# jurmy24/orb-slam3-rust

Measured on AMD Instinct MI355X. Metric: stereo frames/sec ORB extract+match @752x480, higher is better.
Workload: dtype u8; 1 GPU; Synthetic 752x480 stereo, 2000 ORB/frame, extract+match+triangulate (BASELINE configs[1]); n_features=2000, batch_pairs_per_gpu=512, distinct_batches=3, unique_pairs=1536, parallelism=frames sharded, 1 rank(s), no collective

## Files before the change

orb-slam3-rust_amd/csrc/orb_kernels.hip:

```cpp
#include <cfloat>
#include <cmath>

#include "orbx_internal.hpp"

namespace {

#include "orb_pattern_31.inc"

constexpr int EDGE = 31;

__constant__ __attribute__((aligned(16))) signed char c_pattern[256 * 4];

struct XcdMap { unsigned per_img, magic; };
__device__ __forceinline__ bool xcd_decode_at(XcdMap m, int n_img, unsigned L, int& img, int& b) {
  const unsigned x = L & 7u, slot = L >> 3;
  unsigned grp = __umulhi(slot, m.magic);
  unsigned r = slot - grp * m.per_img;
  if (r >= m.per_img) { ++grp; r -= m.per_img; }
  b = (int)r;
  img = (int)(grp * 8u + x);
  return img < n_img;
}
__device__ __forceinline__ bool xcd_decode(XcdMap m, int n_img, int& img, int& b) { return xcd_decode_at(m, n_img, blockIdx.x, img, b); }
static inline XcdMap xcd_map(int per_img) {
// ... 5 lines not shown
                                                    int& pitch) {
  if (l == 0) { pitch = s.l0_pitch; return s.l0 + (size_t)img * s.l0_img_stride; }
  pitch = g.lv[l].pitch;
  return s.pyr + (size_t)img * g.slot_bytes + g.lv[l].off;
}

__global__ __launch_bounds__(256) void copy_l0_kernel(const uint8_t* __restrict__ src, size_t img_stride,
                                                      size_t row_stride, int w, int h, uint8_t* __restrict__ pyr,
                                                      unsigned slot, int pitch) {
  const int img = blockIdx.z;
  const int y = blockIdx.y;
  const uint8_t* s = src + (size_t)img * img_stride + (size_t)y * row_stride;
  uint8_t* d = pyr + (size_t)img * slot + (size_t)y * pitch;
  for (int x = blockIdx.x * 256 + threadIdx.x; x < w; x += gridDim.x * 256) d[x] = s[x];
}

__device__ __forceinline__ unsigned ld_u32(const uint8_t* p);
#ifndef ORBX_RESIZE_ROWS
#define ORBX_RESIZE_ROWS 6
#endif
constexpr int RESIZE_ROWS = ORBX_RESIZE_ROWS;
__device__ __forceinline__ unsigned pack_byte2(unsigned a, unsigned b, unsigned c, unsigned d) {
  return __builtin_amdgcn_perm(b, a, 0x0c0c0602u) | __builtin_amdgcn_perm(d, c, 0x06020c0cu);
}

__device__ __forceinline__ unsigned resize_h(unsigned long long win, int o, unsigned coef) {
  const unsigned pr = (unsigned)(win >> (8 * o));
  return __builtin_amdgcn_udot4(pr, coef, pr & 0xffu, false);
}

constexpr int RZ_LP = 128;
constexpr int rz_src_rows(int rows) { return (16 * rows - 1) * 3 / 2 + 3; }
constexpr int RESIZE_ROWS_SMALL = 2;
#ifndef ORBX_RESIZE_CHAIN
#define ORBX_RESIZE_CHAIN 1
#endif
constexpr int RESIZE_CHAIN = ORBX_RESIZE_CHAIN;
template <int RESIZE_ROWS>
__global__ __launch_bounds__(256) void resize_kernel(OrbSrc s, OrbGeom g, int l, int n_img, XcdMap xm, int tiles_x, int n_tiles,
                                                     const unsigned* __restrict__ xtab,
                                                     const unsigned* __restrict__ ytab) {
  constexpr int RZ_SRC_ROWS = rz_src_rows(RESIZE_ROWS);
  __shared__ __attribute__((aligned(16))) uint8_t st[RZ_SRC_ROWS * RZ_LP + 16];
  int img, chain;
  if (!xcd_decode(xm, n_img, img, chain)) return;
  int sp;
  const uint8_t* src = level_ptr(s, g, img, l - 1, sp);
  const int sh = g.lv[l - 1].h;
  const int w = g.lv[l].w, h = g.lv[l].h, dp = g.lv[l].pitch;
  uint8_t* dst = s.pyr + (size_t)img * g.slot_bytes + g.lv[l].off;
  const int tid = threadIdx.x;
  constexpr int NP = (RZ_SRC_ROWS + 31) / 32;
  struct Tile { int X0, Y0, ax, ncol, sy_lo, nrow, off; };
  uint4 v[NP];
  auto fetch = [&](int tb, Tile& t) {
    const int tby = tb / tiles_x, tbx = tb - tby * tiles_x;
    t.X0 = tbx * 64; t.Y0 = tby * (16 * RESIZE_ROWS);
    const int sx_lo = (int)(xtab[t.X0] >> 16);
    const int xb_last = min((int)(xtab[min(t.X0 + 60, ((w + 3) & ~3) - 4)] >> 16), sp - 8);
    t.ax = min(sx_lo & ~15, sp - 16);
    t.ncol = (xb_last + 8 - t.ax + 15) >> 4;
    t.sy_lo = (int)(ytab[t.Y0] >> 16);
    const int sy_hi = min((int)(ytab[min(t.Y0 + 16 * RESIZE_ROWS - 1, h - 1)] >> 16) + 1, sh - 1);
    t.nrow = sy_hi - t.sy_lo + 1;
    const int c = tid & 7;
    const int cs = min(t.ax + 16 * c, sp - 16);
    t.off = cs - t.ax;
    const uint8_t* gp = src + (unsigned)(__umul24((unsigned)(t.sy_lo + (tid >> 3)), (unsigned)sp) + (unsigned)cs);
    const unsigned gstep = 32u * (unsigned)sp;
#pragma unroll
    for (int k = 0; k < NP; ++k)
      if (c < t.ncol && (tid >> 3) + 32 * k < t.nrow) __builtin_memcpy(&v[k], gp + (unsigned)k * gstep, 16);
  };
  const int tb0 = chain * RESIZE_CHAIN, tb_end = min(tb0 + RESIZE_CHAIN, n_tiles);
  Tile cur, nxt;
  fetch(tb0, cur);
  for (int tb = tb0; tb < tb_end; ++tb) {
    const int x0 = cur.X0 + (tid & 15) * 4;
    const int yb = cur.Y0 + (tid >> 4);
    const bool active = yb < h && x0 < w;
    uint4 xt4 = {0u, 0u, 0u, 0u};
    unsigned yt[RESIZE_ROWS];
    if (active) {
      xt4 = *reinterpret_cast<const uint4*>(xtab + x0);
#pragma unroll
      for (int r = 0; r < RESIZE_ROWS; ++r) yt[r] = ytab[min(yb + 16 * r, h - 1)];
    }
#pragma unroll
    for (int k = 0; k < NP; ++k) {
      const int r = (tid >> 3) + 32 * k;
      if ((tid & 7) < cur.ncol && r < cur.nrow) {
        if ((cur.off & 15) == 0) *reinterpret_cast<uint4*>(&st[r * RZ_LP + cur.off]) = v[k];
        else {
          unsigned* q = reinterpret_cast<unsigned*>(&st[r * RZ_LP + cur.off]);
          q[0] = v[k].x; q[1] = v[k].y; q[2] = v[k].z; q[3] = v[k].w;
        }
      }
    }
    __syncthreads();
    if (tb + 1 < tb_end) fetch(tb + 1, nxt);
    if (active) {
      const unsigned xt[4] = {xt4.x, xt4.y, xt4.z, xt4.w};
      const int xb = min((int)(xt[0] >> 16), sp - 8);
      const int col = xb - cur.ax, sh8 = col & 3;
      const uint8_t* lp = st + (col & ~3);
#pragma unroll
      for (int r = 0; r < RESIZE_ROWS; ++r) {
        const int y = yb + 16 * r;
        if (y >= h) break;
        const int y0 = (int)(yt[r] >> 16), y1 = min(y0 + 1, sh - 1);
        const unsigned* p0 = reinterpret_cast<const unsigned*>(lp + (y0 - cur.sy_lo) * RZ_LP);
        const unsigned* p1 = reinterpret_cast<const unsigned*>(lp + (y1 - cur.sy_lo) * RZ_LP);
        const unsigned a0 = p0[0], a1 = p0[1], a2 = p0[2], b0 = p1[0], b1 = p1[1], b2 = p1[2];
        const unsigned long long w0 = (unsigned long long)__builtin_amdgcn_alignbyte(a1, a0, (unsigned)sh8) |
                                      ((unsigned long long)__builtin_amdgcn_alignbyte(a2, a1, (unsigned)sh8) << 32);
        const unsigned long long w1 = (unsigned long long)__builtin_amdgcn_alignbyte(b1, b0, (unsigned)sh8) |
                                      ((unsigned long long)__builtin_amdgcn_alignbyte(b2, b1, (unsigned)sh8) << 32);
        const unsigned cy1 = yt[r] & 0xffffu, cy0 = 256u - cy1;
        unsigned vv[4];
#pragma unroll
        for (int k = 0; k < 4; ++k) {
          const int o = (int)(xt[k] >> 16) - xb;
          const unsigned cx1 = xt[k] & 0xffffu;
          const unsigned coef = (255u - cx1) | (cx1 << 8);
          const unsigned h0 = resize_h(w0, o, coef), h1 = resize_h(w1, o, coef);
          vv[k] = __umul24(cy0, h0) + __umul24(cy1, h1) + 32768u;
        }
        const unsigned packed = pack_byte2(vv[0], vv[1], vv[2], vv[3]);
        *reinterpret_cast<unsigned*>(dst + (unsigned)(__umul24((unsigned)y, (unsigned)dp) + (unsigned)x0)) = packed;
      }
    }
    __syncthreads();
    cur = nxt;
  }
}

__device__ __forceinline__ void decode_tile(const unsigned* __restrict__ tab, int tile, int& l, int& tx, int& ty) {
  const unsigned e = tab[tile];
  l = (int)(e & 7u); tx = (int)((e >> 3) & 0x3fffu); ty = (int)(e >> 17);
}


#ifndef ORBX_BLUR_PF
#define ORBX_BLUR_PF 2
#endif
constexpr int BLUR_PF = ORBX_BLUR_PF;
#ifndef ORBX_BLUR_STRIP
#define ORBX_BLUR_STRIP 32
#endif
#if defined(ORBX_BLUR_NOARITH) && ORBX_BLUR_NOARITH == 2
constexpr int BLUR_W = 256, BLUR_HALO = 0;
#else
constexpr int BLUR_W = 248, BLUR_HALO = 1;
#endif
constexpr int BLUR_STRIP = ORBX_BLUR_STRIP, BLUR_H = 4 * BLUR_STRIP;

__device__ __forceinline__ void blur_hsum(unsigned d0, unsigned d1, unsigned d2, unsigned (&hs)[4]) {
  const unsigned G0 = 18u | (34u << 8) | (48u << 16) | (56u << 24);
  const unsigned G1 = 48u | (34u << 8) | (18u << 16);
  hs[0] = __builtin_amdgcn_udot4(__builtin_amdgcn_alignbyte(d2, d1, 1), G1,
                                 __builtin_amdgcn_udot4(__builtin_amdgcn_alignbyte(d1, d0, 1), G0, 0u, false), false);
  hs[1] = __builtin_amdgcn_udot4(__builtin_amdgcn_alignbyte(d2, d1, 2), G1,
                                 __builtin_amdgcn_udot4(__builtin_amdgcn_alignbyte(d1, d0, 2), G0, 0u, false), false);
  hs[2] = __builtin_amdgcn_udot4(__builtin_amdgcn_alignbyte(d2, d1, 3), G1,
                                 __builtin_amdgcn_udot4(__builtin_amdgcn_alignbyte(d1, d0, 3), G0, 0u, false), false);
  hs[3] = __builtin_amdgcn_udot4(d2, G1, __builtin_amdgcn_udot4(d1, G0, 0u, false), false);
}
// ... 473 lines not shown
  __syncthreads();
  for (int q = tid; q < npos; q += FT_THREADS) {
    const int p = s_pos[q];
    const int j = p >> 6, i = p & 63;
    const int x = x0 + i - 1, y = y0 + j - 1;
    const int sc = ss[j][i];
    const bool corner = sc > 0 && i >= 1 && i <= FT_W && j >= 1 && j <= FT_H && x < w - EDGE && y < h - EDGE;
    if (corner) {
      const int m = max(max(max((int)ss[j - 1][i - 1], (int)ss[j - 1][i]), max((int)ss[j - 1][i + 1], (int)ss[j][i - 1])),
                        max(max((int)ss[j][i + 1], (int)ss[j + 1][i - 1]), max((int)ss[j + 1][i], (int)ss[j + 1][i + 1])));
      if (sc > m) {
        const int pos = atomicAdd(&s_cnt, 1);
        if (pos < FAST_LIST_CAP) s_list[pos] = ((unsigned)sc << 24) | ((unsigned)y << 12) | (unsigned)x;
        else atomicOr(status, ORBX_ST_INTERNAL);
      }
    }
  }
  __syncthreads();
  acc_cnt = min(s_cnt, FAST_LIST_CAP);
  acc_il = img * g.n_levels + l;
  acc_off = g.lv[l].cand_off;
  acc_cap = g.lv[l].cand_cap;
  cur = nxt;
  }
  if (acc_cnt > 0) append();
}

__device__ __forceinline__ unsigned ld_u32(const uint8_t* p) {
  unsigned v;
  __builtin_memcpy(&v, p, 4);
  return v;
}

__device__ __forceinline__ float harris_response(const uint8_t* __restrict__ img, int pitch, int x0, int y0) {
  int a = 0, b = 0, c = 0;
  int rowm[9], row0[9], rowp[9];
  unsigned w[9][3];
#ifdef ORBX_HARRIS_UNALIGNED
  const uint8_t* p = img + (size_t)(y0 - 4) * pitch + (x0 - 4);
#pragma unroll
  for (int r = 0; r < 9; ++r) {
    const uint8_t* pr = p + (size_t)r * pitch;
    w[r][0] = ld_u32(pr); w[r][1] = ld_u32(pr + 4); w[r][2] = ld_u32(pr + 8);
  }
#else
  const unsigned sh = (unsigned)(x0 - 4) & 3u;
  const uint8_t* p = img + (unsigned)(__umul24((unsigned)(y0 - 4), (unsigned)pitch) + ((unsigned)(x0 - 4) & ~3u));
  struct alignas(4) Row12 { unsigned d[3]; };
  Row12 rw[9];
#pragma unroll
  for (int r = 0; r < 9; ++r) rw[r] = *reinterpret_cast<const Row12*>(p + (unsigned)r * (unsigned)pitch);
#pragma unroll
  for (int r = 0; r < 9; ++r) {
    w[r][0] = __builtin_amdgcn_alignbyte(rw[r].d[1], rw[r].d[0], sh);
    w[r][1] = __builtin_amdgcn_alignbyte(rw[r].d[2], rw[r].d[1], sh);
    w[r][2] = rw[r].d[2] >> (8u * sh);
  }
#endif
#define ORBX_ROW(dst, r)                                                                    \
  _Pragma("unroll") for (int k = 0; k < 4; ++k) {                                             \
    dst[k] = (int)((w[r][0] >> (8 * k)) & 0xffu);                                             \
    dst[4 + k] = (int)((w[r][1] >> (8 * k)) & 0xffu);                                         \
  }                                                                                           \
  dst[8] = (int)(w[r][2] & 0xffu);
  ORBX_ROW(rowm, 0)
  ORBX_ROW(row0, 1)
#pragma unroll
  for (int i = 0; i < 7; ++i) {
    ORBX_ROW(rowp, i + 2)
#pragma unroll
    for (int j = 0; j < 7; ++j) {
      const int Ix = (row0[j + 2] - row0[j]) * 2 + (rowm[j + 2] - rowm[j]) + (rowp[j + 2] - rowp[j]);
      const int Iy = (rowp[j + 1] - rowm[j + 1]) * 2 + (rowp[j] - rowm[j]) + (rowp[j + 2] - rowm[j + 2]);
      a += Ix * Ix; b += Iy * Iy; c += Ix * Iy;
    }
#pragma unroll
    for (int k = 0; k < 9; ++k) { rowm[k] = row0[k]; row0[k] = rowp[k]; }
  }
#undef ORBX_ROW
  const float scale = 1.f / (4 * 7 * 255.f);
  const float scale_sq_sq = scale * scale * scale * scale;
  const float fa = (float)a, fb = (float)b, fc = (float)c;
  const float t1 = __fmul_rn(fa, fb);
  const float t2 = __fmul_rn(fc, fc);
  const float sm = __fadd_rn(fa, fb);
  const float t3 = __fmul_rn(__fmul_rn(0.04f, sm), sm);
  float r = __fmul_rn(__fsub_rn(__fsub_rn(t1, t2), t3), scale_sq_sq);
  if (r == 0.f) r = 0.f;
  return r;
}

__device__ __forceinline__ unsigned orderable(float f) {
  const unsigned u = __float_as_uint(f);
  return (u & 0x80000000u) ? ~u : (u | 0x80000000u);
}
__device__ __forceinline__ float from_orderable(unsigned o) {
  const unsigned u = (o & 0x80000000u) ? (o & 0x7fffffffu) : ~o;
  return __uint_as_float(u);
}

struct HarrisPlan { int start[ORBX_MAX_LEVELS + 1]; };
__global__ __launch_bounds__(256) void harris_select_kernel(OrbSrc s, OrbGeom g, int n_img, XcdMap xm, const unsigned* __restrict__ cand,
                                                            const unsigned* __restrict__ cand_count,
                                                            const unsigned* __restrict__ hist,
                                                            unsigned long long* __restrict__ sel,
                                                            unsigned* __restrict__ sel_count, HarrisPlan hp) {
  __shared__ unsigned sh[256];
  __shared__ int s_thr;
  int img, bb;
  if (!xcd_decode(xm, n_img, img, bb)) return;
  int l = 0;
#pragma unroll
  for (int k = 1; k < ORBX_MAX_LEVELS; ++k) l += (bb >= hp.start[k]) ? 1 : 0;
  const int chunk = bb - hp.start[l], n_chunks = hp.start[l + 1] - hp.start[l];
  const int il = img * g.n_levels + l;
  const int tid = threadIdx.x;
  const unsigned count = min(cand_count[il], g.lv[l].cand_cap);
  const unsigned want = 2u * (unsigned)g.lv[l].quota;
  {
    const int lane = tid & 63, wave = tid >> 6;
    const unsigned hv = hist[(size_t)il * 256 + tid];
    const int incl = wave_scan_incl((int)hv);
    unsigned suf = (unsigned)(__builtin_amdgcn_readlane(incl, 63) - incl) + hv;
    if (lane == 0) sh[wave] = suf;
    if (tid == 0) s_thr = 0;
    __syncthreads();
    for (int w2 = wave + 1; w2 < 4; ++w2) suf += sh[w2];
    const unsigned long long m = __ballot(suf >= want);
    if (want == 0) { if (tid == 0) s_thr = 256; }
    else if (count > want && m && lane == 0) atomicMax(&s_thr, wave * 64 + 63 - __clzll((long long)m));
    __syncthreads();
  }
  const unsigned thr = (unsigned)s_thr;
  int pitch;
  const uint8_t* src = level_ptr(s, g, img, l, pitch);
  const unsigned* cl = cand + (size_t)img * g.cand_total + g.lv[l].cand_off;
  unsigned long long* out = sel + (size_t)img * g.cand_total + g.lv[l].cand_off;
  __shared__ unsigned s_pass[1024];
  __shared__ unsigned s_np;
  const int lane = tid & 63;
  const unsigned per = (count + (unsigned)n_chunks - 1u) / (unsigned)n_chunks;
  const unsigned lim = min(count, (chunk + 1) * per);
  for (unsigned base = chunk * per; base < lim; base += 1024u) {
    if (tid == 0) s_np = 0;
    __syncthreads();
#pragma unroll
    for (int k = 0; k < 4; ++k) {
      const unsigned i = base + k * 256 + tid;
      const unsigned c = i < lim ? cl[i] : 0u;
      const bool pass = i < lim && (c >> 24) >= thr;
      const unsigned long long m = __ballot(pass);
      if (m) {
        unsigned p0 = 0;
        if (lane == 0) p0 = (unsigned)lds_add_rtn(reinterpret_cast<int*>(&s_np), __popcll(m));
        p0 = __builtin_amdgcn_readfirstlane(p0);
        if (pass) s_pass[p0 + __builtin_amdgcn_mbcnt_hi((unsigned)(m >> 32), __builtin_amdgcn_mbcnt_lo((unsigned)m, 0u))] = c;
      }
    }
    __syncthreads();
    const unsigned np = s_np;
    unsigned mine = 0;
    for (unsigned q0 = (unsigned)(tid & ~63); q0 < np; q0 += 256) mine += min(64u, np - q0);
    unsigned pos0 = 0;
    if (lane == 0 && mine) pos0 = atomicAdd(&sel_count[il], mine);
    for (unsigned q0 = 0; q0 < np; q0 += 256) {
      const unsigned q = q0 + tid;
      if (q < np) {
        const unsigned c = s_pass[q];
        const int x = (int)(c & 0xfffu), y = (int)((c >> 12) & 0xfffu);
        const float r = harris_response(src, pitch, x, y);
        const unsigned long long key = ((unsigned long long)(~orderable(r)) << 32) | ((unsigned)y << 16) | (unsigned)x;
        out[__builtin_amdgcn_readfirstlane(pos0) + (q0 >> 8) * 64u + (unsigned)lane] = key;
      }
    }
    __syncthreads();
  }
}

constexpr int RK_NT = 256;
#ifndef ORBX_RK_CAP
#define ORBX_RK_CAP 1024
#endif
constexpr int RK_CAP = ORBX_RK_CAP;
static_assert(RK_CAP == 1024 || RK_CAP == 2048, "a power of two, at least the 1024 counters the tile sort keeps in the array, at most the 2048 keys held in registers");
template <int E>
__device__ __forceinline__ void rank_pass(const unsigned long long* __restrict__ in, unsigned long long* __restrict__ out,
                                          unsigned M, unsigned g0, unsigned long long* chunk, int quota, unsigned* s_thr) {
  constexpr int CH = RK_CAP;
  const int tid = threadIdx.x;
  unsigned long long my[E];
  unsigned rank[E];
#pragma unroll
  for (int e = 0; e < E; ++e) {
    const unsigned idx = g0 + e * RK_NT + tid;
    my[e] = idx < M ? in[idx] : ~0ull;
    rank[e] = 0;
  }
  for (unsigned c0 = 0; c0 < M; c0 += CH) {
    const unsigned n = min((unsigned)CH, M - c0);
    __syncthreads();
    for (unsigned i = tid; i < n; i += RK_NT) chunk[i] = in[c0 + i];
    __syncthreads();
    for (unsigned k = 0; k < n; ++k) {
      const unsigned long long v = chunk[k];
#pragma unroll
      for (int e = 0; e < E; ++e) rank[e] += (v < my[e]) ? 1u : 0u;
// ... 581 lines not shown
      for (int mb = 0; mb < 4; ++mb) a1[mb] = anx[mb] ^ (df_i4){(int)0x80808080u, (int)0x80808080u, (int)0x80808080u, (int)0x80808080u};
      if (wi + 4 < nwin) fetch(wi + 4, anx);
      unsigned char* out0 = s_tile + (unsigned)((c - ox + m16) * DT_PITCH + (r - oy) + 4 * q);
#pragma unroll
      for (int nb = 0; nb < 3; ++nb) {
        const df_i4 t1 = band[64 * nb];
        df_i4 hh[4];
#pragma unroll
        for (int mb = 0; mb < 4; ++mb) hh[mb] = __builtin_amdgcn_mfma_i32_16x16x64_i8(a1[mb], t1, (df_i4){0, 0, 0, 0}, 0, 0, 0);
        df_i4 bhi, blo;
#pragma unroll
        for (int mb = 0; mb < 4; ++mb) {
          const unsigned p01 = __builtin_amdgcn_perm((unsigned)hh[mb][1], (unsigned)hh[mb][0], 0x05010400u);
          const unsigned p23 = __builtin_amdgcn_perm((unsigned)hh[mb][3], (unsigned)hh[mb][2], 0x05010400u);
          blo[mb] = (int)(__builtin_amdgcn_perm(p23, p01, 0x05040100u) ^ 0x80808080u);
          bhi[mb] = (int)__builtin_amdgcn_perm(p23, p01, 0x07060302u);
        }
#pragma unroll
        for (int mb2 = 0; mb2 < 3; ++mb2) {
          const df_i4 t2 = band[64 * (3 + mb2)];
          const df_i4 shi = __builtin_amdgcn_mfma_i32_16x16x64_i8(t2, bhi, (df_i4){0, 0, 0, 0}, 0, 0, 0);
          const df_i4 slo = __builtin_amdgcn_mfma_i32_16x16x64_i8(t2, blo, (df_i4){8454144, 8454144, 8454144, 8454144}, 0, 0, 0);
          const unsigned v0 = ((unsigned)shi[0] << 8) + (unsigned)slo[0], v1 = ((unsigned)shi[1] << 8) + (unsigned)slo[1];
          const unsigned v2 = ((unsigned)shi[2] << 8) + (unsigned)slo[2], v3 = ((unsigned)shi[3] << 8) + (unsigned)slo[3];
          const unsigned u01 = __builtin_amdgcn_perm(v1, v0, 0x00000602u), u23 = __builtin_amdgcn_perm(v3, v2, 0x00000602u);
          *reinterpret_cast<unsigned*>(out0 + (16 * nb) * DT_PITCH + 16 * mb2) = __builtin_amdgcn_perm(u23, u01, 0x05040100u);
        }
      }
    }
  }
  __syncthreads();
  const unsigned astep = 4u * (unsigned)pitch;
  struct alignas(4) Row12 { unsigned d[3]; };
  auto pixels = [&](unsigned long long e, unsigned long long (&px)[8]) {
    const int kx = (int)(e & 0xffffu), ky = (int)((e >> 16) & 0xffffu);
#ifdef ORBX_DT_CENTROID_UNALIGNED
    const uint8_t* a0 = src + (unsigned)(__umul24((unsigned)(ky - 15 + (li >> 2)), (unsigned)pitch) + (unsigned)(kx - 15 + 8 * (li & 3)));
#pragma unroll
    for (int it = 0; it < 8; ++it) {
      const int row = 4 * it + (li >> 2);
      __builtin_memcpy(&px[it], a0 + ((unsigned)it * astep - (row > 30 ? (unsigned)pitch : 0u)), 8);
    }
#else
    const unsigned xb = (unsigned)(kx - 15 + 8 * (li & 3)), sh = xb & 3u;
    unsigned off = __umul24((unsigned)(ky - 15 + (li >> 2)), (unsigned)pitch) + (xb & ~3u);
    Row12 rw[8];
#pragma unroll
    for (int it = 0; it < 8; ++it) {
      rw[it] = *reinterpret_cast<const Row12*>(src + (it == 7 && (li >> 2) == 3 ? off - (unsigned)pitch : off));
      off += astep;
    }
#pragma unroll
    for (int it = 0; it < 8; ++it)
      px[it] = (unsigned long long)__builtin_amdgcn_alignbyte(rw[it].d[1], rw[it].d[0], sh) |
               ((unsigned long long)__builtin_amdgcn_alignbyte(rw[it].d[2], rw[it].d[1], sh) << 32);
#endif
  };
  typedef float desc_f4 __attribute__((ext_vector_type(4)));
  auto centroid = [&](const unsigned long long (&px)[8], int& m10, int& m01) {
    int sA = 0, sB = 0, sC = 0;
#pragma unroll
    for (int it = 0; it < 8; ++it) {
      const int row = 4 * it + (li >> 2);
      const int r = min(row, 30);
      const int t0 = row * 8 + 2 * (li & 3);
      const uint2 w1 = *reinterpret_cast<const uint2*>(&s_ones[t0]);
      const uint2 wc = *reinterpret_cast<const uint2*>(&s_col[t0]);
      const unsigned sI = __builtin_amdgcn_udot4((unsigned)(px[it] >> 32), w1.y, __builtin_amdgcn_udot4((unsigned)px[it], w1.x, 0u, false), false);
      sA += (int)__builtin_amdgcn_udot4((unsigned)(px[it] >> 32), wc.y, __builtin_amdgcn_udot4((unsigned)px[it], wc.x, 0u, false), false);
      sB += (int)sI;
      sC += (r - 15) * (int)sI;
    }
    sA = row16_sum(sA); sB = row16_sum(sB); sC = row16_sum(sC);
    m10 = sA - 15 * sB; m01 = sC;
  };
  const int l32 = lane & 31, hf = lane >> 5;
  unsigned long long e0 = ent, e1 = ent_n, e2 = ent_2, e3 = ent_3;
  for (unsigned g0 = (unsigned)wave; g0 < ngrp; g0 += 16) {
    int sel10, sel01;
    {
      unsigned long long pxa[8], pxb[8];
      int m10, m01;
      pixels(e0, pxa);
      if (g0 + 4 < ngrp) pixels(e1, pxb);
      centroid(pxa, m10, m01);
      sel10 = m10; sel01 = m01;
      if (g0 + 4 < ngrp) {
        if (g0 + 8 < ngrp) pixels(e2, pxa);
        centroid(pxb, m10, m01);
        if (li == 1) { sel10 = m10; sel01 = m01; }
        if (g0 + 8 < ngrp) {
          if (g0 + 12 < ngrp) pixels(e3, pxb);
          centroid(pxa, m10, m01);
          if (li == 2) { sel10 = m10; sel01 = m01; }
          if (g0 + 12 < ngrp) {
            centroid(pxb, m10, m01);
            if (li == 3) { sel10 = m10; sel01 = m01; }
          }
        }
      }
    }
    int pidx = 8 * l32;
    asm volatile("" : "+v"(pidx));
    desc_f4 pat[8];
#pragma unroll
    for (int r = 0; r < 8; ++r) {
      const int pr = s_pat[pidx + r];
      pat[r] = (desc_f4){(float)(signed char)(pr & 0xff), (float)(signed char)((pr >> 16) & 0xff), (float)(signed char)((pr >> 8) & 0xff), (float)(signed char)((pr >> 24) & 0xff)};
    }
    const unsigned long long es = li == 1 ? e1 : li == 2 ? e2 : li == 3 ? e3 : e0;
    const unsigned j2_s = (unsigned)(es >> 32) & 0xffffu;
    const unsigned gi_s = g0 + 4u * (unsigned)(li & 3);
    const int kx_s = (int)(es & 0xffffu), ky_s = (int)((es >> 16) & 0xffffu);
    const unsigned slot_s = lbase + j2_s;
    const bool active_s = li < 4 && gi_s < ngrp && gi_s * DG_PER_WAVE + (unsigned)grp < n_kp && slot_s < limit;
    const float resp = from_orderable(~(unsigned)(sel2[lofs + j2_s] >> 32));
    const unsigned long long n0 = entry(g0 + 16u), n1 = entry(g0 + 20u);
    const float angle16 = fast_atan2_deg((float)sel01, (float)sel10);
    float ca16, sa16;
    sincos_deg(angle16, ca16, sa16);
    constexpr unsigned kBias = 0x400000u * DT_PITCH + 0x4B400000u;
    const unsigned kbase16 = (unsigned)((kx_s - (ox + 3)) * DT_PITCH + (ky_s - (oy + 3))) - kBias;
    const unsigned slot16 = active_s ? slot_s : 0xffffffffu;
    if (active_s) {
      const float sc = g.lv[l].scale;
      orbx_keypoint o;
      o.x = __fmul_rn((float)kx_s, sc);
      o.y = __fmul_rn((float)ky_s, sc);
      o.size = __fmul_rn(patch_size, sc);
      o.angle = angle16;
      o.response = resp;
      o.octave = l;
// ... 243 lines not shown
  if (int rc = orbx_reserve(h, h->ws_sel, sizeof(unsigned long long) * (size_t)g.cand_total * n)) return rc;
  if (int rc = orbx_reserve(h, h->ws_sel2, sizeof(unsigned long long) * (size_t)g.cand_total * n)) return rc;
  if (int rc = orbx_reserve(h, h->ws_dtile, sizeof(uint2) * (size_t)std::max(g.dt_total, 1) * n)) return rc;
  const size_t n_cnt = n_il * (3 + 256);
  if (int rc = orbx_reserve(h, h->ws_counters, sizeof(unsigned) * n_cnt)) return rc;
  ORBX_HIP(h, hipMemsetAsync(h->ws_counters.p, 0, sizeof(unsigned) * n_cnt, st));
  unsigned* cc = (unsigned*)h->ws_counters.p;
  unsigned* sc = cc + n_il;
  unsigned* kp = sc + n_il;
  unsigned* hs = kp + n_il;
  unsigned* cand = (unsigned*)h->ws_cand.p;
  unsigned long long* sel = (unsigned long long*)h->ws_sel.p;
  unsigned long long* sel2 = (unsigned long long*)h->ws_sel2.p;
  uint2* dtile = (uint2*)h->ws_dtile.p;
  const bool aligned = ((uintptr_t)d_images % 4 == 0) && (stride % 4 == 0) && (((size_t)h_px * stride) % 4 == 0);
  const unsigned* tab = (const unsigned*)h->resize_tab.p;
  OrbSrc s{};
  s.pyr = (uint8_t*)h->ws_pyr.p;
  if (aligned) {
    s.l0 = d_images; s.l0_img_stride = (size_t)h_px * stride; s.l0_pitch = (int)stride;
  } else {
    ProfScope ps(h, "copy_l0_kernel");
    hipLaunchKernelGGL(copy_l0_kernel, dim3(1, h_px, n), dim3(256), 0, st, d_images, (size_t)h_px * stride, stride, w, h_px, s.pyr,
                       g.slot_bytes, g.lv[0].pitch);
    s.l0 = s.pyr; s.l0_img_stride = g.slot_bytes; s.l0_pitch = g.lv[0].pitch;
  }
  h->last_src = s; h->last_n_images = n;
  {
    ProfScope ps(h, "resize_kernel");
    for (int l = 1; l < nl; ++l) {
      const bool small = n < 64;
      const int rows = small ? RESIZE_ROWS_SMALL : RESIZE_ROWS;
      const int tx = (g.lv[l].w + 63) / 64, ty = (g.lv[l].h + 16 * rows - 1) / (16 * rows);
      const int chains = (tx * ty + RESIZE_CHAIN - 1) / RESIZE_CHAIN;
      if (small)
        hipLaunchKernelGGL(resize_kernel<RESIZE_ROWS_SMALL>, xcd_grid(chains, n), dim3(256), 0, st, s, g, l, n, xcd_map(chains), tx, tx * ty,
                           tab + h->resize_tab_off[2 * l], tab + h->resize_tab_off[2 * l + 1]);
      else
        hipLaunchKernelGGL(resize_kernel<RESIZE_ROWS>, xcd_grid(chains, n), dim3(256), 0, st, s, g, l, n, xcd_map(chains), tx, tx * ty,
                           tab + h->resize_tab_off[2 * l], tab + h->resize_tab_off[2 * l + 1]);
    }
  }
  if (g.ftiles_total > 0) {
    ProfScope ps(h, "fast_kernel", true);
    const int chain_len = (size_t)g.ftiles_total * n >= (size_t)4 * 8 * h->n_cu ? FAST_CHAIN : 1;
    const int chains = (g.ftiles_total + chain_len - 1) / chain_len;
    if (g.fast_threshold < 128)
      hipLaunchKernelGGL(fast_kernel<true>, xcd_grid(chains, n), dim3(FT_THREADS), 0, st, s, g, n, xcd_map(chains), tab + h->ftile_tab_off, cand, cc, hs, g.ftiles_total, chain_len, h->d_status);
    else
      hipLaunchKernelGGL(fast_kernel<false>, xcd_grid(chains, n), dim3(FT_THREADS), 0, st, s, g, n, xcd_map(chains), tab + h->ftile_tab_off, cand, cc, hs, g.ftiles_total, chain_len, h->d_status);
  }
  {
    ProfScope ps(h, "harris_select_kernel", true);
    HarrisPlan hp{};
    const int hb_total = std::min(512, std::max(16, (40 * h->orb.n_features + 1000) / 2000));
    double area = 0;
    for (int l = 0; l < nl; ++l) area += (double)g.lv[l].w * g.lv[l].h;
    for (int l = 0; l < nl; ++l) hp.start[l + 1] = hp.start[l] + std::max(1, (int)lrint(hb_total * ((double)g.lv[l].w * g.lv[l].h) / area));
    for (int l = nl; l < ORBX_MAX_LEVELS; ++l) hp.start[l + 1] = hp.start[nl];
    const int hblocks = hp.start[nl];
    hipLaunchKernelGGL(harris_select_kernel, xcd_grid(hblocks, n), dim3(256), 0, st, s, g, n, xcd_map(hblocks),
                       (const unsigned*)cand, cc, hs, sel, sc, hp);
  }
  {
    ProfScope ps(h, "rank_select_kernel", true);
    hipLaunchKernelGGL(rank_select_kernel, xcd_grid(nl, n), dim3(RK_NT), 0, st, g, n, xcd_map(nl), sel, sc,
                       sel2, kp, dtile);
  }
  static const bool dt_force = [] { const char* e = getenv("ORBX_DESC_TILE"); return e && atoi(e) == 1; }();
  if (g.dt_total > 0 && (dt_force || (size_t)g.dt_total * (size_t)n >= (size_t)8 * (size_t)h->n_cu)) {
    ProfScope ps(h, "describe_tile_kernel", true);
    hipLaunchKernelGGL(describe_tile_kernel, xcd_grid(g.dt_total, n), dim3(256), 0, st, s, g, n, xcd_map(g.dt_total), tab + h->dtile_tab_off,
                       (const uint2*)dtile, (const unsigned long long*)sel2, (const unsigned long long*)sel, kp, d_kp,
// ... 60 lines not shown
```

Before: 184,600 stereo frames/s.

## Pack resize tile loads into flat pieces and hoist centroid loads ahead

The resize kernel drops its tile chaining and handles one tile per block. Source staging now uses a flat piece index over rows times columns, so all 256 threads issue 16-byte loads instead of a fixed 8-column by 32-row mapping that left lanes idle. Threads with no valid piece write to a dump region of shared memory, which avoids branching on the store. In the descriptor kernel, the centroid row loads are issued as raw words earlier and byte-aligned only when consumed, so more global loads are in flight before the arithmetic; this costs more registers.

New measurement: 186,300 stereo frames/s, median of 6. No clear change (+0.9%).

```diff
diff --git a/orb-slam3-rust_amd/csrc/orb_kernels.hip b/orb-slam3-rust_amd/csrc/orb_kernels.hip
--- a/orb-slam3-rust_amd/csrc/orb_kernels.hip
+++ b/orb-slam3-rust_amd/csrc/orb_kernels.hip
@@ -61,107 +61,110 @@
 constexpr int RZ_LP = 128;
 constexpr int rz_src_rows(int rows) { return (16 * rows - 1) * 3 / 2 + 3; }
 constexpr int RESIZE_ROWS_SMALL = 2;
-#ifndef ORBX_RESIZE_CHAIN
-#define ORBX_RESIZE_CHAIN 1
-#endif
-constexpr int RESIZE_CHAIN = ORBX_RESIZE_CHAIN;
 template <int RESIZE_ROWS>
 __global__ __launch_bounds__(256) void resize_kernel(OrbSrc s, OrbGeom g, int l, int n_img, XcdMap xm, int tiles_x, int n_tiles,
                                                      const unsigned* __restrict__ xtab,
                                                      const unsigned* __restrict__ ytab) {
   constexpr int RZ_SRC_ROWS = rz_src_rows(RESIZE_ROWS);
-  __shared__ __attribute__((aligned(16))) uint8_t st[RZ_SRC_ROWS * RZ_LP + 16];
-  int img, chain;
-  if (!xcd_decode(xm, n_img, img, chain)) return;
+  constexpr int RZ_DUMP = RZ_SRC_ROWS * RZ_LP + 16;
+  __shared__ __attribute__((aligned(16))) uint8_t st[RZ_DUMP + 64 * 16];
+  int img, tb;
+  if (!xcd_decode(xm, n_img, img, tb)) return;
   int sp;
   const uint8_t* src = level_ptr(s, g, img, l - 1, sp);
   const int sh = g.lv[l - 1].h;
   const int w = g.lv[l].w, h = g.lv[l].h, dp = g.lv[l].pitch;
   uint8_t* dst = s.pyr + (size_t)img * g.slot_bytes + g.lv[l].off;
   const int tid = threadIdx.x;
-  constexpr int NP = (RZ_SRC_ROWS + 31) / 32;
-  struct Tile { int X0, Y0, ax, ncol, sy_lo, nrow, off; };
+  constexpr int NP = (RZ_SRC_ROWS * 8 + 255) / 256, NU = NP < 3 ? NP : 3;
+  struct Tile { int X0, Y0, ax, ncol, sy_lo, nrow, npiece, lds[NP]; };
+  struct Tabs { uint4 x; unsigned y[RESIZE_ROWS]; };
   uint4 v[NP];
-  auto fetch = [&](int tb, Tile& t) {
+  const int x_last = ((w + 3) & ~3) - 4;
+  auto tables = [&](int tb, Tile& t, Tabs& e) {
     const int tby = tb / tiles_x, tbx = tb - tby * tiles_x;
     t.X0 = tbx * 64; t.Y0 = tby * (16 * RESIZE_ROWS);
+    e.x = *reinterpret_cast<const uint4*>(xtab + min(t.X0 + (tid & 15) * 4, x_last));
+#pragma unroll
+    for (int r = 0; r < RESIZE_ROWS; ++r) e.y[r] = ytab[min(t.Y0 + (tid >> 4) + 16 * r, h - 1)];
+  };
+  auto fetch = [&](Tile& t) {
     const int sx_lo = (int)(xtab[t.X0] >> 16);
-    const int xb_last = min((int)(xtab[min(t.X0 + 60, ((w + 3) & ~3) - 4)] >> 16), sp - 8);
+    const int xb_last = min((int)(xtab[min(t.X0 + 60, x_last)] >> 16), sp - 8);
     t.ax = min(sx_lo & ~15, sp - 16);
     t.ncol = (xb_last + 8 - t.ax + 15) >> 4;
     t.sy_lo = (int)(ytab[t.Y0] >> 16);
     const int sy_hi = min((int)(ytab[min(t.Y0 + 16 * RESIZE_ROWS - 1, h - 1)] >> 16) + 1, sh - 1);
     t.nrow = sy_hi - t.sy_lo + 1;
-    const int c = tid & 7;
-    const int cs = min(t.ax + 16 * c, sp - 16);
-    t.off = cs - t.ax;
-    const uint8_t* gp = src + (unsigned)(__umul24((unsigned)(t.sy_lo + (tid >> 3)), (unsigned)sp) + (unsigned)cs);
-    const unsigned gstep = 32u * (unsigned)sp;
-#pragma unroll
-    for (int k = 0; k < NP; ++k)
-      if (c < t.ncol && (tid >> 3) + 32 * k < t.nrow) __builtin_memcpy(&v[k], gp + (unsigned)k * gstep, 16);
+    t.npiece = t.nrow * t.ncol;
+    const float rcol = 1.0f / (float)t.ncol;
+    auto piece = [&](int k) {
+      const int i = min(tid + 256 * k, t.npiece - 1);
+      const int r = (int)(((float)i + 0.5f) * rcol), c = i - r * t.ncol;
+      const int cs = min(t.ax + 16 * c, sp - 16);
+      t.lds[k] = r * RZ_LP + (cs - t.ax);
+      __builtin_memcpy(&v[k], src + (unsigned)(__umul24((unsigned)(t.sy_lo + r), (unsigned)sp) + (unsigned)cs), 16);
+    };
+#pragma unroll
+    for (int k = NU; k < NP; ++k)
+      if (256 * k < t.npiece) piece(k);
+#pragma unroll
+    for (int k = 0; k < NU; ++k) piece(k);
   };
-  const int tb0 = chain * RESIZE_CHAIN, tb_end = min(tb0 + RESIZE_CHAIN, n_tiles);
-  Tile cur, nxt;
-  fetch(tb0, cur);
-  for (int tb = tb0; tb < tb_end; ++tb) {
-    const int x0 = cur.X0 + (tid & 15) * 4;
-    const int yb = cur.Y0 + (tid >> 4);
-    const bool active = yb < h && x0 < w;
-    uint4 xt4 = {0u, 0u, 0u, 0u};
-    unsigned yt[RESIZE_ROWS];
-    if (active) {
-      xt4 = *reinterpret_cast<const uint4*>(xtab + x0);
-#pragma unroll
-      for (int r = 0; r < RESIZE_ROWS; ++r) yt[r] = ytab[min(yb + 16 * r, h - 1)];
-    }
-#pragma unroll
-    for (int k = 0; k < NP; ++k) {
-      const int r = (tid >> 3) + 32 * k;
-      if ((tid & 7) < cur.ncol && r < cur.nrow) {
-        if ((cur.off & 15) == 0) *reinterpret_cast<uint4*>(&st[r * RZ_LP + cur.off]) = v[k];
-        else {
-          unsigned* q = reinterpret_cast<unsigned*>(&st[r * RZ_LP + cur.off]);
-          q[0] = v[k].x; q[1] = v[k].y; q[2] = v[k].z; q[3] = v[k].w;
-        }
-      }
-    }
-    __syncthreads();
-    if (tb + 1 < tb_end) fetch(tb + 1, nxt);
-    if (active) {
-      const unsigned xt[4] = {xt4.x, xt4.y, xt4.z, xt4.w};
-      const int xb = min((int)(xt[0] >> 16), sp - 8);
-      const int col = xb - cur.ax, sh8 = col & 3;
-      const uint8_t* lp = st + (col & ~3);
-#pragma unroll
-      for (int r = 0; r < RESIZE_ROWS; ++r) {
-        const int y = yb + 16 * r;
-        if (y >= h) break;
-        const int y0 = (int)(yt[r] >> 16), y1 = min(y0 + 1, sh - 1);
-        const unsigned* p0 = reinterpret_cast<const unsigned*>(lp + (y0 - cur.sy_lo) * RZ_LP);
-        const unsigned* p1 = reinterpret_cast<const unsigned*>(lp + (y1 - cur.sy_lo) * RZ_LP);
-        const unsigned a0 = p0[0], a1 = p0[1], a2 = p0[2], b0 = p1[0], b1 = p1[1], b2 = p1[2];
-        const unsigned long long w0 = (unsigned long long)__builtin_amdgcn_alignbyte(a1, a0, (unsigned)sh8) |
-                                      ((unsigned long long)__builtin_amdgcn_alignbyte(a2, a1, (unsigned)sh8) << 32);
-        const unsigned long long w1 = (unsigned long long)__builtin_amdgcn_alignbyte(b1, b0, (unsigned)sh8) |
-                                      ((unsigned long long)__builtin_amdgcn_alignbyte(b2, b1, (unsigned)sh8) << 32);
-        const unsigned cy1 = yt[r] & 0xffffu, cy0 = 256u - cy1;
-        unsigned vv[4];
-#pragma unroll
-        for (int k = 0; k < 4; ++k) {
-          const int o = (int)(xt[k] >> 16) - xb;
-          const unsigned cx1 = xt[k] & 0xffffu;
-          const unsigned coef = (255u - cx1) | (cx1 << 8);
-          const unsigned h0 = resize_h(w0, o, coef), h1 = resize_h(w1, o, coef);
-          vv[k] = __umul24(cy0, h0) + __umul24(cy1, h1) + 32768u;
-        }
-        const unsigned packed = pack_byte2(vv[0], vv[1], vv[2], vv[3]);
-        *reinterpret_cast<unsigned*>(dst + (unsigned)(__umul24((unsigned)y, (unsigned)dp) + (unsigned)x0)) = packed;
-      }
-    }
-    __syncthreads();
-    cur = nxt;
-  }
+  auto stage = [&](const Tile& t) {
+    const int dump = RZ_DUMP + 16 * (tid & 63);
+    if (sp & 15) {
+#pragma unroll
+      for (int k = 0; k < NP; ++k) {
+        unsigned* q = reinterpret_cast<unsigned*>(st + (tid + 256 * k < t.npiece ? t.lds[k] : dump));
+        q[0] = v[k].x; q[1] = v[k].y; q[2] = v[k].z; q[3] = v[k].w;
+      }
+    } else {
+#pragma unroll
+      for (int k = 0; k < NP; ++k) *reinterpret_cast<uint4*>(st + (tid + 256 * k < t.npiece ? t.lds[k] : dump)) = v[k];
+    }
+  };
+  auto compute = [&](const Tile& t, const Tabs& e) {
+    const int x0 = t.X0 + (tid & 15) * 4;
+    const int yb = t.Y0 + (tid >> 4);
+    if (yb >= h || x0 >= w) return;
+    const unsigned xt[4] = {e.x.x, e.x.y, e.x.z, e.x.w};
+    const int xb = min((int)(xt[0] >> 16), sp - 8);
+    const int col = xb - t.ax, sh8 = col & 3;
+    const uint8_t* lp = st + (col & ~3);
+#pragma unroll
+    for (int r = 0; r < RESIZE_ROWS; ++r) {
+      const int y = yb + 16 * r;
+      if (y >= h) break;
+      const int y0 = (int)(e.y[r] >> 16), y1 = min(y0 + 1, sh - 1);
+      const unsigned* p0 = reinterpret_cast<const unsigned*>(lp + (y0 - t.sy_lo) * RZ_LP);
+      const unsigned* p1 = reinterpret_cast<const unsigned*>(lp + (y1 - t.sy_lo) * RZ_LP);
+      const unsigned a0 = p0[0], a1 = p0[1], a2 = p0[2], b0 = p1[0], b1 = p1[1], b2 = p1[2];
+      const unsigned long long w0 = (unsigned long long)__builtin_amdgcn_alignbyte(a1, a0, (unsigned)sh8) |
+                                    ((unsigned long long)__builtin_amdgcn_alignbyte(a2, a1, (unsigned)sh8) << 32);
+      const unsigned long long w1 = (unsigned long long)__builtin_amdgcn_alignbyte(b1, b0, (unsigned)sh8) |
+                                    ((unsigned long long)__builtin_amdgcn_alignbyte(b2, b1, (unsigned)sh8) << 32);
+      const unsigned cy1 = e.y[r] & 0xffffu, cy0 = 256u - cy1;
+      unsigned vv[4];
+#pragma unroll
+      for (int k = 0; k < 4; ++k) {
+        const int o = (int)(xt[k] >> 16) - xb;
+        const unsigned cx1 = xt[k] & 0xffffu;
+        const unsigned coef = (255u - cx1) | (cx1 << 8);
+        const unsigned h0 = resize_h(w0, o, coef), h1 = resize_h(w1, o, coef);
+        vv[k] = __umul24(cy0, h0) + __umul24(cy1, h1) + 32768u;
+      }
+      const unsigned packed = pack_byte2(vv[0], vv[1], vv[2], vv[3]);
+      *reinterpret_cast<unsigned*>(dst + (unsigned)(__umul24((unsigned)y, (unsigned)dp) + (unsigned)x0)) = packed;
+    }
+  };
+  Tile t;
+  Tabs e;
+  tables(tb, t, e);
+  fetch(t);
+  stage(t);
+  __syncthreads();
+  compute(t, e);
 }
 
 __device__ __forceinline__ void decode_tile(const unsigned* __restrict__ tab, int tile, int& l, int& tx, int& ty) {
@@ -1488,42 +1491,32 @@
   __syncthreads();
   const unsigned astep = 4u * (unsigned)pitch;
   struct alignas(4) Row12 { unsigned d[3]; };
-  auto pixels = [&](unsigned long long e, unsigned long long (&px)[8]) {
+  struct Round { Row12 rw[8]; unsigned sh; };
+  auto request = [&](unsigned long long e, Round& rd) {
     const int kx = (int)(e & 0xffffu), ky = (int)((e >> 16) & 0xffffu);
-#ifdef ORBX_DT_CENTROID_UNALIGNED
-    const uint8_t* a0 = src + (unsigned)(__umul24((unsigned)(ky - 15 + (li >> 2)), (unsigned)pitch) + (unsigned)(kx - 15 + 8 * (li & 3)));
+    const unsigned xb = (unsigned)(kx - 15 + 8 * (li & 3));
+    rd.sh = xb & 3u;
+    unsigned off = __umul24((unsigned)(ky - 15 + (li >> 2)), (unsigned)pitch) + (xb & ~3u);
 #pragma unroll
     for (int it = 0; it < 8; ++it) {
-      const int row = 4 * it + (li >> 2);
-      __builtin_memcpy(&px[it], a0 + ((unsigned)it * astep - (row > 30 ? (unsigned)pitch : 0u)), 8);
-    }
-#else
-    const unsigned xb = (unsigned)(kx - 15 + 8 * (li & 3)), sh = xb & 3u;
-    unsigned off = __umul24((unsigned)(ky - 15 + (li >> 2)), (unsigned)pitch) + (xb & ~3u);
-    Row12 rw[8];
-#pragma unroll
-    for (int it = 0; it < 8; ++it) {
-      rw[it] = *reinterpret_cast<const Row12*>(src + (it == 7 && (li >> 2) == 3 ? off - (unsigned)pitch : off));
+      rd.rw[it] = *reinterpret_cast<const Row12*>(src + (it == 7 && (li >> 2) == 3 ? off - (unsigned)pitch : off));
       off += astep;
     }
-#pragma unroll
-    for (int it = 0; it < 8; ++it)
-      px[it] = (unsigned long long)__builtin_amdgcn_alignbyte(rw[it].d[1], rw[it].d[0], sh) |
-               ((unsigned long long)__builtin_amdgcn_alignbyte(rw[it].d[2], rw[it].d[1], sh) << 32);
-#endif
   };
   typedef float desc_f4 __attribute__((ext_vector_type(4)));
-  auto centroid = [&](const unsigned long long (&px)[8], int& m10, int& m01) {
+  auto centroid = [&](const Round& rd, int& m10, int& m01) {
     int sA = 0, sB = 0, sC = 0;
 #pragma unroll
     for (int it = 0; it < 8; ++it) {
+      const unsigned long long pxi = (unsigned long long)__builtin_amdgcn_alignbyte(rd.rw[it].d[1], rd.rw[it].d[0], rd.sh) |
+                                     ((unsigned long long)__builtin_amdgcn_alignbyte(rd.rw[it].d[2], rd.rw[it].d[1], rd.sh) << 32);
       const int row = 4 * it + (li >> 2);
       const int r = min(row, 30);
       const int t0 = row * 8 + 2 * (li & 3);
       const uint2 w1 = *reinterpret_cast<const uint2*>(&s_ones[t0]);
       const uint2 wc = *reinterpret_cast<const uint2*>(&s_col[t0]);
-      const unsigned sI = __builtin_amdgcn_udot4((unsigned)(px[it] >> 32), w1.y, __builtin_amdgcn_udot4((unsigned)px[it], w1.x, 0u, false), false);
-      sA += (int)__builtin_amdgcn_udot4((unsigned)(px[it] >> 32), wc.y, __builtin_amdgcn_udot4((unsigned)px[it], wc.x, 0u, false), false);
+      const unsigned sI = __builtin_amdgcn_udot4((unsigned)(pxi >> 32), w1.y, __builtin_amdgcn_udot4((unsigned)pxi, w1.x, 0u, false), false);
+      sA += (int)__builtin_amdgcn_udot4((unsigned)(pxi >> 32), wc.y, __builtin_amdgcn_udot4((unsigned)pxi, wc.x, 0u, false), false);
       sB += (int)sI;
       sC += (r - 15) * (int)sI;
     }
@@ -1535,25 +1528,20 @@
   for (unsigned g0 = (unsigned)wave; g0 < ngrp; g0 += 16) {
     int sel10, sel01;
     {
-      unsigned long long pxa[8], pxb[8];
+      Round ra, rb;
       int m10, m01;
-      pixels(e0, pxa);
-      if (g0 + 4 < ngrp) pixels(e1, pxb);
-      centroid(pxa, m10, m01);
-      sel10 = m10; sel01 = m01;
-      if (g0 + 4 < ngrp) {
-        if (g0 + 8 < ngrp) pixels(e2, pxa);
-        centroid(pxb, m10, m01);
+      request(e0, ra);
+      request(e1, rb);
+      centroid(ra, sel10, sel01);
+      if (g0 + 8 >= ngrp) {
+        if (g0 + 4 < ngrp) { centroid(rb, m10, m01); if (li == 1) { sel10 = m10; sel01 = m01; } }
+      } else {
+        request(e2, ra);
+        centroid(rb, m10, m01);
         if (li == 1) { sel10 = m10; sel01 = m01; }
-        if (g0 + 8 < ngrp) {
-          if (g0 + 12 < ngrp) pixels(e3, pxb);
-          centroid(pxa, m10, m01);
-          if (li == 2) { sel10 = m10; sel01 = m01; }
-          if (g0 + 12 < ngrp) {
-            centroid(pxb, m10, m01);
-            if (li == 3) { sel10 = m10; sel01 = m01; }
-          }
-        }
+        centroid(ra, m10, m01);
+        if (li == 2) { sel10 = m10; sel01 = m01; }
+        if (g0 + 12 < ngrp) { request(e3, rb); centroid(rb, m10, m01); if (li == 3) { sel10 = m10; sel01 = m01; } }
       }
     }
     int pidx = 8 * l32;
@@ -1863,13 +1851,9 @@
       const bool small = n < 64;
       const int rows = small ? RESIZE_ROWS_SMALL : RESIZE_ROWS;
       const int tx = (g.lv[l].w + 63) / 64, ty = (g.lv[l].h + 16 * rows - 1) / (16 * rows);
-      const int chains = (tx * ty + RESIZE_CHAIN - 1) / RESIZE_CHAIN;
-      if (small)
-        hipLaunchKernelGGL(resize_kernel<RESIZE_ROWS_SMALL>, xcd_grid(chains, n), dim3(256), 0, st, s, g, l, n, xcd_map(chains), tx, tx * ty,
-                           tab + h->resize_tab_off[2 * l], tab + h->resize_tab_off[2 * l + 1]);
-      else
-        hipLaunchKernelGGL(resize_kernel<RESIZE_ROWS>, xcd_grid(chains, n), dim3(256), 0, st, s, g, l, n, xcd_map(chains), tx, tx * ty,
-                           tab + h->resize_tab_off[2 * l], tab + h->resize_tab_off[2 * l + 1]);
+      const auto kern = small ? resize_kernel<RESIZE_ROWS_SMALL> : resize_kernel<RESIZE_ROWS>;
+      hipLaunchKernelGGL(kern, xcd_grid(tx * ty, n), dim3(256), 0, st, s, g, l, n, xcd_map(tx * ty), tx, tx * ty,
+                         tab + h->resize_tab_off[2 * l], tab + h->resize_tab_off[2 * l + 1]);
     }
   }
   if (g.ftiles_total > 0) {
```

## Cooperatively stage Harris windows in LDS and batch survivor compaction

Applied to the files above, without the earlier changes.

The Harris select kernel now has all 256 threads gather the 9-row, 12-byte windows of up to 128 survivors into shared memory, with one row load per thread per pass. Only the first two waves then compute responses from LDS, instead of every thread issuing nine strided global loads. Candidate loads are hoisted before the barrier, and the four per-wave LDS atomics are merged into one. Occupancy is hinted with launch_bounds(256,8). The trade-off is fewer threads doing the arithmetic, an extra barrier per sub-batch, and 13.5KB of extra LDS.

Result: no change. 184,000 stereo frames/s before, 183,700 stereo frames/s after (-0.2%).

```diff
diff --git a/orb-slam3-rust_amd/csrc/orb_kernels.hip b/orb-slam3-rust_amd/csrc/orb_kernels.hip
--- a/orb-slam3-rust_amd/csrc/orb_kernels.hip
+++ b/orb-slam3-rust_amd/csrc/orb_kernels.hip
@@ -701,37 +701,19 @@
   return v;
 }
 
-__device__ __forceinline__ float harris_response(const uint8_t* __restrict__ img, int pitch, int x0, int y0) {
+__device__ __forceinline__ float harris_response(const unsigned* rw, unsigned sh) {
   int a = 0, b = 0, c = 0;
   int rowm[9], row0[9], rowp[9];
-  unsigned w[9][3];
-#ifdef ORBX_HARRIS_UNALIGNED
-  const uint8_t* p = img + (size_t)(y0 - 4) * pitch + (x0 - 4);
-#pragma unroll
-  for (int r = 0; r < 9; ++r) {
-    const uint8_t* pr = p + (size_t)r * pitch;
-    w[r][0] = ld_u32(pr); w[r][1] = ld_u32(pr + 4); w[r][2] = ld_u32(pr + 8);
-  }
-#else
-  const unsigned sh = (unsigned)(x0 - 4) & 3u;
-  const uint8_t* p = img + (unsigned)(__umul24((unsigned)(y0 - 4), (unsigned)pitch) + ((unsigned)(x0 - 4) & ~3u));
-  struct alignas(4) Row12 { unsigned d[3]; };
-  Row12 rw[9];
-#pragma unroll
-  for (int r = 0; r < 9; ++r) rw[r] = *reinterpret_cast<const Row12*>(p + (unsigned)r * (unsigned)pitch);
-#pragma unroll
-  for (int r = 0; r < 9; ++r) {
-    w[r][0] = __builtin_amdgcn_alignbyte(rw[r].d[1], rw[r].d[0], sh);
-    w[r][1] = __builtin_amdgcn_alignbyte(rw[r].d[2], rw[r].d[1], sh);
-    w[r][2] = rw[r].d[2] >> (8u * sh);
-  }
-#endif
 #define ORBX_ROW(dst, r)                                                                    \
-  _Pragma("unroll") for (int k = 0; k < 4; ++k) {                                             \
-    dst[k] = (int)((w[r][0] >> (8 * k)) & 0xffu);                                             \
-    dst[4 + k] = (int)((w[r][1] >> (8 * k)) & 0xffu);                                         \
-  }                                                                                           \
-  dst[8] = (int)(w[r][2] & 0xffu);
+  {                                                                                           \
+    const unsigned d0 = rw[3 * (r)], d1 = rw[3 * (r) + 1], d2 = rw[3 * (r) + 2];              \
+    const unsigned w0 = __builtin_amdgcn_alignbyte(d1, d0, sh), w1 = __builtin_amdgcn_alignbyte(d2, d1, sh), w2 = d2 >> (8u * sh); \
+    _Pragma("unroll") for (int k = 0; k < 4; ++k) {                                           \
+      dst[k] = (int)((w0 >> (8 * k)) & 0xffu);                                                \
+      dst[4 + k] = (int)((w1 >> (8 * k)) & 0xffu);                                            \
+    }                                                                                         \
+    dst[8] = (int)(w2 & 0xffu);                                                               \
+  }
   ORBX_ROW(rowm, 0)
   ORBX_ROW(row0, 1)
 #pragma unroll
@@ -768,8 +750,10 @@
   return __uint_as_float(u);
 }
 
+constexpr int HS_SUB = 128;
+static_assert(HS_SUB % 64 == 0 && HS_SUB <= 256, "whole waves of survivors");
 struct HarrisPlan { int start[ORBX_MAX_LEVELS + 1]; };
-__global__ __launch_bounds__(256) void harris_select_kernel(OrbSrc s, OrbGeom g, int n_img, XcdMap xm, const unsigned* __restrict__ cand,
+__global__ __launch_bounds__(256, 8) void harris_select_kernel(OrbSrc s, OrbGeom g, int n_img, XcdMap xm, const unsigned* __restrict__ cand,
                                                             const unsigned* __restrict__ cand_count,
                                                             const unsigned* __restrict__ hist,
                                                             unsigned long long* __restrict__ sel,
@@ -786,6 +770,9 @@
   const int tid = threadIdx.x;
   const unsigned count = min(cand_count[il], g.lv[l].cand_cap);
   const unsigned want = 2u * (unsigned)g.lv[l].quota;
+  const unsigned* cl = cand + (size_t)img * g.cand_total + g.lv[l].cand_off;
+  const unsigned per = (count + (unsigned)n_chunks - 1u) / (unsigned)n_chunks;
+  const unsigned lim = min(count, (chunk + 1) * per);
   {
     const int lane = tid & 63, wave = tid >> 6;
     const unsigned hv = hist[(size_t)il * 256 + tid];
@@ -803,44 +790,71 @@
   const unsigned thr = (unsigned)s_thr;
   int pitch;
   const uint8_t* src = level_ptr(s, g, img, l, pitch);
-  const unsigned* cl = cand + (size_t)img * g.cand_total + g.lv[l].cand_off;
   unsigned long long* out = sel + (size_t)img * g.cand_total + g.lv[l].cand_off;
   __shared__ unsigned s_pass[1024];
+  __shared__ unsigned s_win[HS_SUB * 27];
   __shared__ unsigned s_np;
-  const int lane = tid & 63;
-  const unsigned per = (count + (unsigned)n_chunks - 1u) / (unsigned)n_chunks;
-  const unsigned lim = min(count, (chunk + 1) * per);
+  const int lane = tid & 63, wave = tid >> 6;
   for (unsigned base = chunk * per; base < lim; base += 1024u) {
+    unsigned cv[4];
+#pragma unroll
+    for (int k = 0; k < 4; ++k) cv[k] = cl[min(base + k * 256 + tid, lim - 1u)];
     if (tid == 0) s_np = 0;
     __syncthreads();
+    unsigned long long m[4];
+    unsigned tot = 0;
 #pragma unroll
     for (int k = 0; k < 4; ++k) {
-      const unsigned i = base + k * 256 + tid;
-      const unsigned c = i < lim ? cl[i] : 0u;
-      const bool pass = i < lim && (c >> 24) >= thr;
-      const unsigned long long m = __ballot(pass);
-      if (m) {
-        unsigned p0 = 0;
-        if (lane == 0) p0 = (unsigned)lds_add_rtn(reinterpret_cast<int*>(&s_np), __popcll(m));
-        p0 = __builtin_amdgcn_readfirstlane(p0);
-        if (pass) s_pass[p0 + __builtin_amdgcn_mbcnt_hi((unsigned)(m >> 32), __builtin_amdgcn_mbcnt_lo((unsigned)m, 0u))] = c;
+      m[k] = __ballot(base + k * 256 + tid < lim && (cv[k] >> 24) >= thr);
+      tot += (unsigned)__popcll(m[k]);
+    }
+    if (tot) {
+      unsigned p0 = 0;
+      if (lane == 0) p0 = (unsigned)lds_add_rtn(reinterpret_cast<int*>(&s_np), (int)tot);
+      p0 = __builtin_amdgcn_readfirstlane(p0);
+#pragma unroll
+      for (int k = 0; k < 4; ++k) {
+        if ((m[k] >> lane) & 1ull)
+          s_pass[p0 + __builtin_amdgcn_mbcnt_hi((unsigned)(m[k] >> 32), __builtin_amdgcn_mbcnt_lo((unsigned)m[k], 0u))] = cv[k];
+        p0 += (unsigned)__popcll(m[k]);
       }
     }
     __syncthreads();
     const unsigned np = s_np;
     unsigned mine = 0;
-    for (unsigned q0 = (unsigned)(tid & ~63); q0 < np; q0 += 256) mine += min(64u, np - q0);
+    if (wave * 64 < HS_SUB)
+      for (unsigned q = (unsigned)(wave * 64); q < np; q += HS_SUB) mine += min(64u, np - q);
     unsigned pos0 = 0;
-    if (lane == 0 && mine) pos0 = atomicAdd(&sel_count[il], mine);
-    for (unsigned q0 = 0; q0 < np; q0 += 256) {
-      const unsigned q = q0 + tid;
-      if (q < np) {
-        const unsigned c = s_pass[q];
-        const int x = (int)(c & 0xfffu), y = (int)((c >> 12) & 0xfffu);
-        const float r = harris_response(src, pitch, x, y);
-        const unsigned long long key = ((unsigned long long)(~orderable(r)) << 32) | ((unsigned)y << 16) | (unsigned)x;
-        out[__builtin_amdgcn_readfirstlane(pos0) + (q0 >> 8) * 64u + (unsigned)lane] = key;
-      }
+    unsigned lane_zero;
+    asm("v_mov_b32 %0, 0" : "=v"(lane_zero));
+    for (unsigned q0 = 0; q0 < np; q0 += HS_SUB) {
+      const unsigned n = min((unsigned)HS_SUB, np - q0);
+      struct alignas(4) Row12 { unsigned d[3]; };
+      constexpr int PASSES = (HS_SUB * 9 + 255) / 256;
+      Row12 rw[PASSES];
+#pragma unroll
+      for (int i = 0; i < PASSES; ++i) {
+        const unsigned t = min((unsigned)(i * 256 + tid), n * 9u - 1u);
+        const unsigned sv = t / 9u, r = t - sv * 9u;
+        const unsigned c = s_pass[q0 + sv];
+        const unsigned x = c & 0xfffu, y = (c >> 12) & 0xfffu;
+        rw[i] = *reinterpret_cast<const Row12*>(src + (__umul24(y - 4u + r, (unsigned)pitch) + ((x - 4u) & ~3u)));
+      }
+      if (q0 == 0 && lane == 0 && mine) pos0 = atomicAdd(&sel_count[il] + lane_zero, mine);
+#pragma unroll
+      for (int i = 0; i < PASSES; ++i) {
+        const unsigned t = min((unsigned)(i * 256 + tid), n * 9u - 1u);
+        s_win[3 * t] = rw[i].d[0]; s_win[3 * t + 1] = rw[i].d[1]; s_win[3 * t + 2] = rw[i].d[2];
+      }
+      __syncthreads();
+      if ((unsigned)tid < n) {
+        const unsigned c = s_pass[q0 + tid];
+        const unsigned x = c & 0xfffu, y = (c >> 12) & 0xfffu;
+        const float r = harris_response(s_win + tid * 27, (x - 4u) & 3u);
+        const unsigned long long key = ((unsigned long long)(~orderable(r)) << 32) | (y << 16) | x;
+        out[__builtin_amdgcn_readfirstlane(pos0) + (q0 / HS_SUB) * 64u + (unsigned)lane] = key;
+      }
+      if (q0 + HS_SUB < np) __syncthreads();
     }
     __syncthreads();
   }
```
